# CAS-CLab/quantized-cnn

Measured on AMD Instinct MI355X. Metric: images/sec AlexNet quantized forward, higher is better.
Workload: dtype f32

## Files before the change

include/qcnn_hip.h:

```cpp
#ifndef QCNN_HIP_H_
#define QCNN_HIP_H_

#include <stddef.h>
#include <stdint.h>

#ifdef __cplusplus
extern "C" {
#endif

#define QCNN_ABI_VERSION 5

#define QCNN_SMALL_BATCH_MAX 3

typedef struct QcnnCtx QcnnCtx;

enum { QCNN_CONV = 0, QCNN_POOL = 1, QCNN_FCNT = 2, QCNN_RELU = 3, QCNN_LORN = 4, QCNN_DRPT = 5, QCNN_SMAX = 6 };

typedef struct {
  int type;
  int padSiz, knlSiz, knlCnt, grpCnt, stride, nodCnt, lrnSiz;
  float lrnAlp, lrnBet, lrnIni, drpRat;
} QcnnLayerDesc;

enum {
  QCNN_OPT_LUT_MODE = 0,
  QCNN_OPT_KEEP_ALL = 1,
  QCNN_OPT_PROFILE = 2,
  QCNN_OPT_SMALL_BATCH = 4,
  QCNN_OPT_SPLIT = 5,
  QCNN_OPT_SLIDE = 7,
  QCNN_OPT_DECODE = 8,
  QCNN_OPT_SYM = 9,
  QCNN_OPT_SYM8 = 10,
  QCNN_OPT_PACKED_FC = 11,
  QCNN_OPT_DIRECT_DEC = 12,
  QCNN_OPT_HALF8 = 13,
  QCNN_OPT_DEC_BF16SPLIT = 14,
  QCNN_OPT_HOST_CHUNK = 6,
  QCNN_OPT_STREAMS = 3
};

int qcnn_ctx_create(int device_id, void* stream, QcnnCtx** out);
int qcnn_ctx_destroy(QcnnCtx* ctx);
const char* qcnn_last_error(const QcnnCtx* ctx);
int qcnn_abi_version(void);
int qcnn_device_count(int* count);
int qcnn_set_option(QcnnCtx* ctx, int option, int value);
int qcnn_sync(QcnnCtx* ctx);
int qcnn_ctx_device(const QcnnCtx* ctx);
void* qcnn_ctx_stream(const QcnnCtx* ctx);

int qcnn_model_begin(QcnnCtx* ctx, int layer_cnt, const QcnnLayerDesc* layers, int in_c, int in_h, int in_w);
int qcnn_model_set_layer_shape(QcnnCtx* ctx, int layer, int M, int K, int Cs);
int qcnn_model_set_layer_dense(QcnnCtx* ctx, int layer);
int qcnn_model_set_layer_weights(QcnnCtx* ctx, int layer, const float* bias, const float* weights_file);
int qcnn_quantize_layer(QcnnCtx* ctx, int Ct, int Cin, int kh, int kw, int M, int K, int Cs, const float* weights_host,
                        const float* ctrd_init_host, int max_iter, float* ctrd_out_host, uint8_t* asmt_out_host, double* sse2,
                        int* iters2);
int qcnn_calib_gram(QcnnCtx* ctx, int H, int W, int Cin_total, int grp, int kh, int kw, int stride, int pad,
                    const float* in_nhwc_host, int n, double* gram_inout_host, int accumulate);
int qcnn_quantize_layer_ec(QcnnCtx* ctx, int Ct, int Cin, int grp, int kh, int kw, int M, int K, int Cs, const float* weights_host,
                           const double* gram_host, const float* ctrd_init_host, const uint8_t* asmt_init_host, int sweeps,
                           double ridge, float* ctrd_out_host, uint8_t* asmt_out_host, double* obj_trace, int* changed_trace);
int qcnn_calib_begin(QcnnCtx* ctx, const int* layers, int n_layers);
int qcnn_calib_arm(QcnnCtx* ctx, int on);
int qcnn_calib_read(QcnnCtx* ctx, int layer, double* gram_host, long long* rows);
int qcnn_calib_end(QcnnCtx* ctx);
int qcnn_model_arena_bytes(QcnnCtx* ctx, size_t* bytes);
int qcnn_model_commit(QcnnCtx* ctx, int max_batch, void* dev_arena);
int qcnn_model_arena_ptr(QcnnCtx* ctx, void** dev_ptr, size_t* bytes);
int qcnn_model_arena_checksum(QcnnCtx* ctx, unsigned long long* sum2);
int qcnn_model_set_layer_params(QcnnCtx* ctx, int layer, const float* bias, const float* ctrd_file,
                                const uint8_t* asmt_file);
int qcnn_model_set_layer_params_cbn(QcnnCtx* ctx, int layer, const float* bias, const float* ctrd_file,
                                    const uint8_t* cbn_blocks, size_t cbn_bytes, int bits);
int qcnn_model_mark_loaded(QcnnCtx* ctx);
int qcnn_fm_dims(QcnnCtx* ctx, int l, int* hwc3);

int qcnn_forward(QcnnCtx* ctx, const float* in_nchw_dev, int n, float* prob_dev, uint16_t* top5_dev);
int qcnn_forward_u8(QcnnCtx* ctx, const uint8_t* in_u8_dev, int src_h, int src_w, const float* mean_dev, int n,
                    float* prob_dev, uint16_t* top5_dev);
#define QCNN_MAX_VIEWS 32
typedef struct { int oy, ox, flip; } QcnnView;
int qcnn_views_ten_crop(int src_h, int src_w, int in_h, int in_w, QcnnView* views10);
int qcnn_forward_u8_views(QcnnCtx* ctx, const uint8_t* in_u8_dev, int src_h, int src_w, const float* mean_dev, int n,
                          const QcnnView* views_host, int n_views, float* prob_dev, uint16_t* top5_dev,
                          float* prob_views_dev );
typedef struct { uint64_t offset; int32_t h, w; } QcnnSrcImage;
int qcnn_forward_u8_resized_views(QcnnCtx* ctx, const uint8_t* src_dev, size_t src_bytes,
                                  const QcnnSrcImage* imgs_host, int n, int full_h, int full_w,
                                  const float* mean_dev ,
                                  const QcnnView* views_host, int n_views,
                                  float* prob_dev, uint16_t* top5_dev, float* prob_views_dev);
int qcnn_relaxed_full_size(int h, int w, int full_h, int full_w, int* hf, int* wf, float* scale);
typedef struct { int ay, ax, dy, dx, flip; } QcnnAnchorView;
int qcnn_views_ten_crop_anchored(QcnnAnchorView* views10);
int qcnn_forward_u8_relaxed_views(QcnnCtx* ctx, const uint8_t* src_dev, size_t src_bytes, const QcnnSrcImage* imgs_host, int n,
                                  int full_h, int full_w, const float* mean_crop_dev ,
                                  const QcnnAnchorView* views_host, int n_views,
                                  float* prob_dev, uint16_t* top5_dev, float* prob_views_dev);
typedef struct {
  uint64_t offset;
  int64_t  row_stride;
  int32_t  h, w;
  int32_t  pix_stride;
  int32_t  ch_offset[4];
} QcnnSrcPixels;
int qcnn_src_planar(const QcnnSrcImage* img, int C, QcnnSrcPixels* out);
int qcnn_src_bmp(const uint8_t* file_host, size_t file_bytes, uint64_t file_offset, QcnnSrcPixels* out);
int qcnn_forward_u8_resized_views_strided(QcnnCtx* ctx, const uint8_t* src_dev, size_t src_bytes,
                                          const QcnnSrcPixels* imgs_host, int n, int full_h, int full_w,
                                          const float* mean_dev ,
                                          const QcnnView* views_host, int n_views,
                                          float* prob_dev, uint16_t* top5_dev, float* prob_views_dev);
int qcnn_forward_u8_relaxed_views_strided(QcnnCtx* ctx, const uint8_t* src_dev, size_t src_bytes,
                                          const QcnnSrcPixels* imgs_host, int n, int full_h, int full_w,
                                          const float* mean_crop_dev ,
                                          const QcnnAnchorView* views_host, int n_views,
                                          float* prob_dev, uint16_t* top5_dev, float* prob_views_dev);
enum { QCNN_YUV_JFIF = 0, QCNN_YUV_BT601 = 1, QCNN_YUV_BT709 = 2 };
typedef struct {
  uint64_t y_offset, cb_offset, cr_offset;
  int64_t  y_row_stride, c_row_stride;
  int32_t  h, w;
  int32_t  y_pix_stride, c_pix_stride;
  int32_t  sub_y, sub_x;
  int32_t  matrix;
} QcnnSrcYuv;
enum { QCNN_YUV_NV12 = 0, QCNN_YUV_NV21 = 1, QCNN_YUV_I420 = 2, QCNN_YUV_YV12 = 3, QCNN_YUV_I444 = 4, QCNN_YUV_YUY2 = 5, QCNN_YUV_UYVY = 6 };
int qcnn_src_yuv_frame(int format, uint64_t frame_offset, int h, int w, int64_t pitch, int matrix, QcnnSrcYuv* out);
// ... 85 lines not shown
```

quantized-cnn_amd/capi.py:

```python
from __future__ import annotations

import ctypes as C
import os
import re

PKG = os.path.dirname(os.path.abspath(__file__))
LIB_PATH = os.environ.get("QCNN_HIP_LIB") or os.path.join(PKG, "libqcnn_hip.so")
HEADER_PATH = os.path.join(os.path.dirname(PKG), "include", "qcnn_hip.h")

OPT_LUT_MODE, OPT_KEEP_ALL, OPT_PROFILE, OPT_STREAMS, OPT_SMALL_BATCH, OPT_SPLIT, OPT_HOST_CHUNK, OPT_SLIDE, OPT_DECODE, OPT_SYM, OPT_SYM8, OPT_PACKED_FC, OPT_DIRECT_DEC, OPT_HALF8, OPT_DEC_BF16SPLIT = 0, 1, 2, 3, 4, 5, 6, 7, 8, 9, 10, 11, 12, 13, 14
LUT_EXACT, LUT_MFMA, LUT_MFMA_F16, LUT_MFMA_F16ACC = 0, 1, 2, 3
SMALL_BATCH_MAX = 3


class QcnnLayerDesc(C.Structure):
    _fields_ = [("type", C.c_int), ("padSiz", C.c_int), ("knlSiz", C.c_int), ("knlCnt", C.c_int),
                ("grpCnt", C.c_int), ("stride", C.c_int), ("nodCnt", C.c_int), ("lrnSiz", C.c_int),
                ("lrnAlp", C.c_float), ("lrnBet", C.c_float), ("lrnIni", C.c_float), ("drpRat", C.c_float)]


MAX_VIEWS = 32


class QcnnView(C.Structure):
# ... 27 lines not shown
    _fields_ = [("src_host", C.c_void_p), ("src_bytes", C.c_size_t), ("imgs", C.POINTER(QcnnSrcPixels)), ("n", C.c_int),
                ("labels", C.c_void_p), ("prob_host", C.c_void_p), ("top5_host", C.c_void_p), ("prob_views_host", C.c_void_p)]


class QcnnU8YuvBatch(C.Structure):
    _fields_ = [("src_host", C.c_void_p), ("src_bytes", C.c_size_t), ("imgs", C.POINTER(QcnnSrcYuv)), ("n", C.c_int),
                ("labels", C.c_void_p), ("prob_host", C.c_void_p), ("top5_host", C.c_void_p), ("prob_views_host", C.c_void_p)]


def layer_desc(ly: dict) -> QcnnLayerDesc:
    return QcnnLayerDesc(ly["type"], ly.get("pad", 0), ly.get("knl", 0), ly.get("cnt", 0), ly.get("grp", 0),
                         ly.get("stride", 0), ly.get("nod", 0), ly.get("siz", 0), ly.get("alp", 0.0),
                         ly.get("bet", 0.0), ly.get("ini", 0.0), ly.get("rat", 0.0))


def declared_symbols():
    txt = open(HEADER_PATH).read()
    txt = re.sub(r"/\*.*?\*/", "", txt, flags=re.S)
    return sorted(set(re.findall(r"\b(qcnn_[a-z0-9_]+)\s*\(", txt)))


_lib = None


def load():
    global _lib
    if _lib is not None:
        return _lib
    if not os.path.exists(LIB_PATH):
        raise RuntimeError("%s is missing: run `python -c 'import __graft_entry__ as g; g.build()'` "
                           "(hipcc --offload-arch=gfx950); there is no fallback path" % LIB_PATH)
    lib = C.CDLL(LIB_PATH)
    vp, i, f32p, u8p, u16p = C.c_void_p, C.c_int, C.c_void_p, C.c_void_p, C.c_void_p
    lib.qcnn_abi_version.restype = i
    lib.qcnn_device_count.argtypes = [C.POINTER(i)]
    lib.qcnn_last_error.restype = C.c_char_p
    lib.qcnn_last_error.argtypes = [vp]
    lib.qcnn_ctx_create.argtypes = [i, vp, C.POINTER(vp)]
    lib.qcnn_ctx_destroy.argtypes = [vp]
    lib.qcnn_set_option.argtypes = [vp, i, i]
    lib.qcnn_sync.argtypes = [vp]
    lib.qcnn_model_begin.argtypes = [vp, i, C.POINTER(QcnnLayerDesc), i, i, i]
    lib.qcnn_model_set_layer_shape.argtypes = [vp, i, i, i, i]
    lib.qcnn_model_set_layer_dense.argtypes = [vp, i]
    lib.qcnn_model_set_layer_weights.argtypes = [vp, i, f32p, f32p]
    lib.qcnn_group_model_set_layer_dense.argtypes = [vp, i]
    lib.qcnn_group_model_set_layer_weights.argtypes = [vp, i, f32p, f32p]
    lib.qcnn_model_arena_bytes.argtypes = [vp, C.POINTER(C.c_size_t)]
    lib.qcnn_model_commit.argtypes = [vp, i, vp]
    lib.qcnn_model_set_layer_params.argtypes = [vp, i, f32p, f32p, u8p]
    lib.qcnn_model_set_layer_params_cbn.argtypes = [vp, i, f32p, f32p, u8p, C.c_size_t, i]
    lib.qcnn_model_mark_loaded.argtypes = [vp]
    lib.qcnn_fm_dims.argtypes = [vp, i, C.POINTER(i)]
    lib.qcnn_forward.argtypes = [vp, f32p, i, f32p, u16p]
    lib.qcnn_forward_u8.argtypes = [vp, u8p, i, i, f32p, i, f32p, u16p]
    lib.qcnn_views_ten_crop.argtypes = [i, i, i, i, C.POINTER(QcnnView)]
    lib.qcnn_forward_u8_views.argtypes = [vp, u8p, i, i, f32p, i, C.POINTER(QcnnView), i, f32p, u16p, f32p]
    lib.qcnn_forward_u8_resized_views.argtypes = [vp, u8p, C.c_size_t, C.POINTER(QcnnSrcImage), i, i, i, f32p, C.POINTER(QcnnView), i,
                                                  f32p, u16p, f32p]
    lib.qcnn_views_ten_crop_anchored.argtypes = [C.POINTER(QcnnAnchorView)]
    lib.qcnn_relaxed_full_size.argtypes = [i, i, i, i, C.POINTER(i), C.POINTER(i), C.POINTER(C.c_float)]
    lib.qcnn_forward_u8_relaxed_views.argtypes = [vp, u8p, C.c_size_t, C.POINTER(QcnnSrcImage), i, i, i, f32p, C.POINTER(QcnnAnchorView), i,
                                                  f32p, u16p, f32p]
    lib.qcnn_src_planar.argtypes = [C.POINTER(QcnnSrcImage), i, C.POINTER(QcnnSrcPixels)]
    lib.qcnn_src_bmp.argtypes = [C.c_char_p, C.c_size_t, C.c_uint64, C.POINTER(QcnnSrcPixels)]
    lib.qcnn_forward_u8_resized_views_strided.argtypes = [vp, u8p, C.c_size_t, C.POINTER(QcnnSrcPixels), i, i, i, f32p,
                                                          C.POINTER(QcnnView), i, f32p, u16p, f32p]
    lib.qcnn_forward_u8_relaxed_views_strided.argtypes = [vp, u8p, C.c_size_t, C.POINTER(QcnnSrcPixels), i, i, i, f32p,
                                                          C.POINTER(QcnnAnchorView), i, f32p, u16p, f32p]
    lib.qcnn_src_yuv_frame.argtypes = [i, C.c_uint64, i, i, C.c_int64, i, C.POINTER(QcnnSrcYuv)]
    lib.qcnn_forward_u8_resized_views_yuv.argtypes = [vp, u8p, C.c_size_t, C.POINTER(QcnnSrcYuv), i, i, i, f32p, C.POINTER(QcnnView), i,
                                                      f32p, u16p, f32p]
    lib.qcnn_forward_u8_relaxed_views_yuv.argtypes = [vp, u8p, C.c_size_t, C.POINTER(QcnnSrcYuv), i, i, i, f32p,
                                                      C.POINTER(QcnnAnchorView), i, f32p, u16p, f32p]
    lib.qcnn_forward_host.argtypes = [vp, f32p, i, f32p, u16p]
    lib.qcnn_forward_host_batches.argtypes = [vp, C.POINTER(vp), C.POINTER(i), i, C.POINTER(vp), C.POINTER(vp)]
    lib.qcnn_forward_u8_resized_host_batches.argtypes = [vp, C.POINTER(QcnnU8Batch), i, i, i, f32p, C.POINTER(QcnnView), i,
                                                         C.POINTER(C.c_ulonglong)]
    lib.qcnn_forward_u8_relaxed_host_batches.argtypes = [vp, C.POINTER(QcnnU8Batch), i, i, i, f32p, C.POINTER(QcnnAnchorView), i,
                                                         C.POINTER(C.c_ulonglong)]
    lib.qcnn_forward_u8_resized_host_batches_yuv.argtypes = [vp, C.POINTER(QcnnU8YuvBatch), i, i, i, f32p, C.POINTER(QcnnView), i,
                                                             C.POINTER(C.c_ulonglong)]
    lib.qcnn_forward_u8_relaxed_host_batches_yuv.argtypes = [vp, C.POINTER(QcnnU8YuvBatch), i, i, i, f32p, C.POINTER(QcnnAnchorView), i,
                                                             C.POINTER(C.c_ulonglong)]
    lib.qcnn_count_top5_hits.argtypes = [vp, u16p, u16p, i, vp]
    lib.qcnn_host_register.argtypes = [vp, C.c_size_t]
    lib.qcnn_host_unregister.argtypes = [vp]
    lib.qcnn_host_alloc.argtypes = [C.c_size_t, C.POINTER(vp)]
    lib.qcnn_host_free.argtypes = [vp]
    lib.qcnn_get_layer_output.argtypes = [vp, i, i, f32p]
    lib.qcnn_get_layer_output_range.argtypes = [vp, i, i, i, f32p]
    lib.qcnn_run_layer.argtypes = [vp, i, f32p, i, f32p]
    lib.qcnn_get_layer_split.argtypes = [vp, i, C.POINTER(i), C.POINTER(i)]
    lib.qcnn_get_layer_dec_form.argtypes = [vp, i, C.POINTER(i), C.POINTER(C.c_longlong)]
    lib.qcnn_get_layer_segments.argtypes = [vp, i, C.POINTER(i), C.POINTER(i)]
    lib.qcnn_get_layer_ms.argtypes = [vp, C.POINTER(C.c_float), C.POINTER(i)]
    lib.qcnn_reset_layer_ms.argtypes = [vp]
    lib.qcnn_get_layer_total_ms.argtypes = [vp, C.POINTER(C.c_double), C.POINTER(C.c_longlong), C.POINTER(i)]
    lib.qcnn_ctx_device.argtypes = [vp]
    lib.qcnn_ctx_stream.argtypes = [vp]
    lib.qcnn_ctx_stream.restype = vp
    lib.qcnn_model_arena_ptr.argtypes = [vp, C.POINTER(vp), C.POINTER(C.c_size_t)]
    lib.qcnn_model_arena_checksum.argtypes = [vp, C.POINTER(C.c_ulonglong)]
    lib.qcnn_quantize_layer.argtypes = [vp, i, i, i, i, i, i, i, f32p, f32p, i, f32p, u8p, C.POINTER(C.c_double), C.POINTER(i)]
    lib.qcnn_calib_gram.argtypes = [vp, i, i, i, i, i, i, i, i, f32p, i, vp, i]
    lib.qcnn_calib_begin.argtypes = [vp, C.POINTER(i), i]
# ... 28 lines not shown
```

quantized-cnn_amd/csrc/qcnn_engine_run.hip:

```cpp
#include <stdlib.h>
#include <string.h>

#include <algorithm>

#include "qcnn_engine.h"

using namespace qcnn_engine;

namespace {

bool decoded_layer(const QcnnCtx* c, int l) {
  const LayerShape& s = c->shapes[l];
  return c->decode && s.decKp > 0 && !s.dense && c->lutMode == 1 && c->layers[l].type == QCNN_CONV;
}

int launched(QcnnCtx* c, int l, hipError_t e) {
  if (e != hipSuccess) return fail(c, "layer %d (type %d) launch failed: %s", l, c->layers[l].type, hipGetErrorString(e));
  return 0;
}

float* conv_partial(QcnnCtx* c, const Launch& L) {
  float* all = ensure_conv_partial(c);
  return all ? all + kConvPartialFloats / (size_t)L.nsub * L.sub : nullptr;
}
// ... 353 lines not shown
      if (prof) {
        HIP_TRY(c, hipEventRecord(e1, st));
        c->profPending.push_back(QcnnCtx::ProfRec{(((size_t)c->profCount * kMaxStreams + k) * c->L + l) * 2, l});
      }
    }
  }
  for (int k = 1; k < ns; ++k) {
    HIP_TRY(c, hipEventRecord(c->evJoin[k - 1], c->aux[k - 1]));
    HIP_TRY(c, hipStreamWaitEvent(c->stream, c->evJoin[k - 1], 0));
  }
  if (c->calib.armed && calib_enqueue(c, fm, n, pa, pb)) return 1;
  if (prof) c->profCount++;
  if (pa == 0 || (int)c->lastFm.size() != c->L + 1) {
    c->lastFm = fm;
  } else {
    for (int l = 0; l <= c->L; ++l)
      if (fm[l] == nullptr) c->lastFm[l] = nullptr;
  }
  c->lastN = n;
  return 0;
}

int map_outputs(QcnnCtx* c, const float* map, int n, float* prob_dev, uint16_t* top5_dev) {
  const int classes = (int)fm_elems(c, c->L);
  hipError_t e;
  if (prob_dev) {
    e = qk_unpack_rows(map, prob_dev, n, classes, c->stream);
    if (e != hipSuccess) return fail(c, "output unpack launch failed: %s", hipGetErrorString(e));
  }
  if (top5_dev) {
    e = qk_top5(map, top5_dev, n, classes, c->stream);
    if (e != hipSuccess) return fail(c, "top-5 launch failed: %s", hipGetErrorString(e));
  }
  return 0;
}
int forward_outputs(QcnnCtx* c, int n, float* prob_dev, uint16_t* top5_dev) {
  return map_outputs(c, c->lastFm[c->L], n, prob_dev, top5_dev);
}
int forward_tail(QcnnCtx* c, int n, float* prob_dev, uint16_t* top5_dev, const float* inNchw) {
  if (run_layers(c, n, inNchw)) return 1;
  return forward_outputs(c, n, prob_dev, top5_dev);
}

}

extern "C" {

int qcnn_fm_dims(QcnnCtx* c, int l, int* hwc3) {
  if (l < 0 || l > c->L) return fail(c, "feature map %d out of range", l);
  hwc3[0] = c->dims[l].h; hwc3[1] = c->dims[l].w; hwc3[2] = c->dims[l].c;
  return 0;
}

int qcnn_forward(QcnnCtx* c, const float* in_nchw_dev, int n, float* prob_dev, uint16_t* top5_dev) {
  if (open_batch(c, n)) return 1;
  if (direct_input(c, n)) return forward_tail(c, n, prob_dev, top5_dev, in_nchw_dev);
  hipError_t e = qk_pack_nchw(in_nchw_dev, c->fmBuf[0], n, c->inC, c->inH, c->inW, c->stream);
  if (e != hipSuccess) return fail(c, "input pack launch failed: %s", hipGetErrorString(e));
  return forward_tail(c, n, prob_dev, top5_dev);
}

int qcnn_forward_u8(QcnnCtx* c, const uint8_t* in_u8_dev, int src_h, int src_w, const float* mean_dev, int n,
                    float* prob_dev, uint16_t* top5_dev) {
  if (open_batch(c, n)) return 1;
  if (src_h < c->inH || src_w < c->inW)
    return fail(c, "source images %dx%d are smaller than the network input %dx%d", src_h, src_w, c->inH, c->inW);
  hipError_t e = qk_pack_u8(in_u8_dev, mean_dev, c->fmBuf[0], n, c->inC, c->inH, c->inW, src_h, src_w, c->stream);
  if (e != hipSuccess) return fail(c, "input pack launch failed: %s", hipGetErrorString(e));
  return forward_tail(c, n, prob_dev, top5_dev);
}

int qcnn_get_layer_output(QcnnCtx* c, int l, int n, float* host_out) {
  HIP_TRY(c, hipSetDevice(c->device));
  if (l < 0 || l > c->L) return fail(c, "feature map %d out of range", l);
  if (n <= 0 || n > c->lastN) return fail(c, "n = %d exceeds the last forward's batch %d", n, c->lastN);
  if (layer_output_ok(c, l)) return 1;
  if (ensure_stage(c, (size_t)n * fm_elems(c, l))) return 1;
  const int E = (int)fm_elems(c, l);
  hipError_t e = qk_unpack_rows(c->lastFm[l], c->stageOut, n, E, c->stream);
  if (e != hipSuccess) return fail(c, "unpack launch failed: %s", hipGetErrorString(e));
  HIP_TRY(c, hipMemcpyAsync(host_out, c->stageOut, (size_t)n * E * sizeof(float), hipMemcpyDeviceToHost, c->stream));
  HIP_TRY(c, hipStreamSynchronize(c->stream));
  return 0;
}

int qcnn_get_layer_output_range(QcnnCtx* c, int l, int first, int n, float* host_out) {
  HIP_TRY(c, hipSetDevice(c->device));
  if (l < 0 || l > c->L) return fail(c, "feature map %d out of range", l);
  if (first < 0 || n <= 0 || first + n > c->lastN)
    return fail(c, "images [%d, %d) are not inside the last forward's batch of %d", first, first + n, c->lastN);
  if (layer_output_ok(c, l)) return 1;
  if (ensure_stage(c, (size_t)(n + QCNN_PANEL) * fm_elems(c, l))) return 1;
  const size_t E = fm_elems(c, l);
  const int p0 = first / QCNN_PANEL;
  const int cnt = first + n - p0 * QCNN_PANEL;
  hipError_t e = qk_unpack_rows(c->lastFm[l] + (size_t)p0 * E * QCNN_PANEL, c->stageOut, cnt, (int)E, c->stream);
  if (e != hipSuccess) return fail(c, "unpack launch failed: %s", hipGetErrorString(e));
  HIP_TRY(c, hipMemcpyAsync(host_out, c->stageOut + (size_t)(first - p0 * QCNN_PANEL) * E, (size_t)n * E * sizeof(float),
                            hipMemcpyDeviceToHost, c->stream));
  HIP_TRY(c, hipStreamSynchronize(c->stream));
  return 0;
}

int qcnn_run_layer(QcnnCtx* c, int layer, const float* in_host, int n, float* out_host) {
  HIP_TRY(c, hipSetDevice(c->device));
  if (!c->committed) return fail(c, "model not committed");
// ... 98 lines not shown
```

quantized-cnn_amd/csrc/qcnn_glue.hip:

```cpp
#include "qcnn_kernels.h"

#include <float.h>
#include <limits.h>

#include <algorithm>

typedef float f32x2 __attribute__((ext_vector_type(2)));
typedef float f32x4 __attribute__((ext_vector_type(4)));

namespace {

constexpr int PANEL = QCNN_PANEL;

__global__ void k_permute_rows(const float* __restrict__ src, float* __restrict__ dst, const int* __restrict__ map,
                               int D, int panels, int livePairs) {
  const int lane = threadIdx.x & 63;
  if (lane >= livePairs) return;
  const size_t rows = (size_t)panels * D;
  for (size_t r = blockIdx.x * (size_t)(blockDim.x >> 6) + (threadIdx.x >> 6); r < rows;
       r += (size_t)gridDim.x * (blockDim.x >> 6)) {
    const size_t panel = r / D;
    const int e = (int)(r % D);
    *reinterpret_cast<f32x2*>(dst + r * PANEL + 2 * lane) =
        *reinterpret_cast<const f32x2*>(src + (panel * D + map[e]) * PANEL + 2 * lane);
  }
}

__global__ void k_sum_partials(const float4* __restrict__ partial, float4* __restrict__ dst, int msplit, size_t n4,
                               int relu) {
  for (size_t i = blockIdx.x * (size_t)blockDim.x + threadIdx.x; i < n4; i += (size_t)gridDim.x * blockDim.x) {
    float4 v = partial[i];
    for (int z = 1; z < msplit; ++z) {
      const float4 w = partial[(size_t)z * n4 + i];
      v.x += w.x; v.y += w.y; v.z += w.z; v.w += w.w;
    }
    if (relu) {
      v.x = (0.0f < v.x) ? v.x : 0.0f;
      v.y = (0.0f < v.y) ? v.y : 0.0f;
      v.z = (0.0f < v.z) ? v.z : 0.0f;
      v.w = (0.0f < v.w) ? v.w : 0.0f;
    }
    dst[i] = v;
  }
}

__global__ void k_relu(const float4* __restrict__ src, float4* __restrict__ dst, size_t n4) {
  for (size_t i = blockIdx.x * (size_t)blockDim.x + threadIdx.x; i < n4; i += (size_t)gridDim.x * blockDim.x) {
    float4 v = src[i];
    v.x = (0.0f < v.x) ? v.x : 0.0f;
    v.y = (0.0f < v.y) ? v.y : 0.0f;
    v.z = (0.0f < v.z) ? v.z : 0.0f;
    v.w = (0.0f < v.w) ? v.w : 0.0f;
    dst[i] = v;
  }
}

template <bool B34>
__device__ __forceinline__ float lrn_scale(float s, float nbet) {
  if (B34) {
    const float r = __builtin_amdgcn_rsqf(s);
    return __fmul_rn(r, __builtin_amdgcn_sqrtf(r));
  }
  return expf(__fmul_rn(nbet, logf(s)));
}

// ... 90 lines not shown
    const int wL = max(0, wo * stride - pad), wU = min(W, wo * stride + knl - pad) - 1;
    const float* base = src + (size_t)panel * H * W * C * PANEL + 2 * lane;
    f32x2 v = {0.0f, 0.0f};
    bool first = true;
    for (int h = hL; h <= hU; ++h)
      for (int w = wL; w <= wU; ++w) {
        const f32x2 s = *reinterpret_cast<const f32x2*>(base + ((size_t)(h * W + w) * C + c) * PANEL);
        if (first) {
          v = s;
        } else {
          v.x = (s.x < v.x) ? v.x : s.x;
          v.y = (s.y < v.y) ? v.y : s.y;
        }
        first = false;
      }
    *reinterpret_cast<f32x2*>(dst + r * PANEL + 2 * lane) = v;
  }
}

__global__ __launch_bounds__(256) void k_pool4(const float4* __restrict__ src, float4* __restrict__ dst, int panels,
                                               int H, int W, int C, int Ho, int Wo, int knl, int stride, int pad,
                                               int liveQuads, int qlShift) {
  const size_t rows = (size_t)panels * Ho * Wo * C;
  const size_t r = (blockIdx.x * (size_t)blockDim.x + threadIdx.x) >> qlShift;
  const int q = threadIdx.x & ((1 << qlShift) - 1);
  if (r >= rows || q >= liveQuads) return;
  const int c = (int)(r % C);
  size_t t = r / C;
  const int wo = (int)(t % Wo);
  t /= Wo;
  const int ho = (int)(t % Ho);
  const int panel = (int)(t / Ho);
  const int hL = max(0, ho * stride - pad), hU = min(H, ho * stride + knl - pad) - 1;
  const int wL = max(0, wo * stride - pad), wU = min(W, wo * stride + knl - pad) - 1;
  const float4* base = src + (size_t)panel * H * W * C * 32 + q;
  float4 v = make_float4(0.0f, 0.0f, 0.0f, 0.0f);
  bool first = true;
  for (int h = hL; h <= hU; ++h)
    for (int w = wL; w <= wU; ++w) {
      const float4 sv = base[((size_t)(h * W + w) * C + c) * 32];
      if (first) {
        v = sv;
      } else {
        v.x = (sv.x < v.x) ? v.x : sv.x;
        v.y = (sv.y < v.y) ? v.y : sv.y;
        v.z = (sv.z < v.z) ? v.z : sv.z;
        v.w = (sv.w < v.w) ? v.w : sv.w;
      }
      first = false;
    }
  dst[r * 32 + q] = v;
}

#ifndef QCNN_LP_PREFETCH
#define QCNN_LP_PREFETCH 0
#endif
#ifndef QCNN_LP_PT
#define QCNN_LP_PT 4
#define QCNN_LP_Q 8
#define QCNN_LP_THREADS 704
#endif
constexpr int LP_PT = QCNN_LP_PT;
constexpr int LP_IT = (LP_PT - 1) * 2 + 3;
constexpr int LP_PIX = LP_IT * LP_IT;
constexpr int LP_Q = QCNN_LP_Q;
constexpr int LP_THREADS = QCNN_LP_THREADS;
template <int N, bool B34>
__global__ __launch_bounds__(LP_THREADS, QCNN_LP_PREFETCH ? 2 : 1) void k_lrn_pool(const float4* __restrict__ src, float4* __restrict__ dst, int H,
                                                         int W, int C, int Ho, int Wo, int tilesX, float coeff, float nbet,
                                                         float ini, int liveQuads) {
  constexpr int RAD = (N - 1) / 2;
  __shared__ float4 slab[N * LP_PIX * LP_Q];
  const int q = threadIdx.x & (LP_Q - 1), rest = threadIdx.x / LP_Q;
  const int slices = 32 / LP_Q;
  const int slice = blockIdx.x % slices, tile = blockIdx.x / slices;
  const int panel = blockIdx.y;
  const int qg = slice * LP_Q + q;
  const bool qlive = qg < liveQuads;
  const int ty = tile / tilesX, tx = tile % tilesX;
  const int ph = ty * LP_PT * 2 + rest / LP_IT, pw = tx * LP_PT * 2 + rest % LP_IT;
  const bool lrnOn = rest < LP_PIX && ph < H && pw < W && qlive;
  const float4* __restrict__ x = src + ((size_t)panel * H * W + (size_t)(lrnOn ? ph * W + pw : 0)) * C * 32 + qg;
  const int pu = rest % N, po = rest / N;
  const int ho = ty * LP_PT + po / LP_PT, wo = tx * LP_PT + po % LP_PT;
  const bool poolOn = po < LP_PT * LP_PT && ho < Ho && wo < Wo && qlive;
  const int hU = min(H, ho * 2 + 3) - 1 - ty * LP_PT * 2, wU = min(W, wo * 2 + 3) - 1 - tx * LP_PT * 2;
  const int hL = (po / LP_PT) * 2, wL = (po % LP_PT) * 2;
  float4* __restrict__ y = dst + ((size_t)panel * Ho * Wo + (size_t)(poolOn ? ho * Wo + wo : 0)) * C * 32 + qg;

  const f32x4 zero = {0.0f, 0.0f, 0.0f, 0.0f};
  f32x4 raw[N], sq[N];
#pragma unroll
  for (int j = 0; j < N; ++j) { raw[j] = zero; sq[j] = zero; }
#pragma unroll
  for (int d = -RAD; d < RAD; ++d) {
    const bool on = lrnOn && d >= 0 && d < C;
    const f32x4 v = ld4(x + (size_t)(on ? d : 0) * 32, on);
    raw[(d + N) % N] = v;
    sq[(d + N) % N] = lrn_sq(v, coeff);
  }
  f32x4* __restrict__ slab4 = reinterpret_cast<f32x4*>(slab);
#if QCNN_LP_PREFETCH
  f32x4 nxt[N];
#pragma unroll
  for (int u = 0; u < N; ++u) nxt[u] = ld4(x + (size_t)(u + RAD < C ? u + RAD : 0) * 32, lrnOn && u + RAD < C);
#endif
  for (int c0 = 0; c0 < C; c0 += N) {
    if (lrnOn) {
#pragma unroll
      for (int u = 0; u < N; ++u) {
        const int c = c0 + u;
        const int tin = c + RAD;
#if QCNN_LP_PREFETCH
        const f32x4 v = nxt[u];
        {
          const int tn = c0 + N + u + RAD;
          nxt[u] = ld4(x + (size_t)(tn < C ? tn : 0) * 32, tn < C);
        }
#else
        const f32x4 v = ld4(x + (size_t)(tin < C ? tin : 0) * 32, tin < C);
#endif
        raw[(u + RAD) % N] = v;
        sq[(u + RAD) % N] = lrn_sq(v, coeff);
        if (c < C) {
          f32x4 sacc = {ini, ini, ini, ini};
#pragma unroll
          for (int j = 0; j < N; ++j) sacc = sacc + sq[(u - RAD + j + N) % N];
          slab4[(u * LP_PIX + rest) * LP_Q + q] = lrn_out<B34>(raw[u % N], sacc, nbet);
        }
      }
    }
    __syncthreads();
    if (poolOn && c0 + pu < C) {
      float4 v = make_float4(0.0f, 0.0f, 0.0f, 0.0f);
      bool first = true;
      for (int h = hL; h <= hU; ++h)
        for (int w = wL; w <= wU; ++w) {
          const float4 sv = slab[(pu * LP_PIX + h * LP_IT + w) * LP_Q + q];
          if (first) {
            v = sv;
          } else {
            v.x = (sv.x < v.x) ? v.x : sv.x;
            v.y = (sv.y < v.y) ? v.y : sv.y;
            v.z = (sv.z < v.z) ? v.z : sv.z;
            v.w = (sv.w < v.w) ? v.w : sv.w;
          }
          first = false;
        }
      y[(size_t)(c0 + pu) * 32] = v;
    }
    __syncthreads();
  }
}

constexpr int SM_LD = 33;
__global__ __launch_bounds__(1024) void k_softmax_lds(const float* __restrict__ src, float* __restrict__ dst, int C) {
  extern __shared__ __attribute__((aligned(16))) char lds[];
  float* tile = reinterpret_cast<float*>(lds);
  float* sums = tile + (size_t)C * SM_LD;
  const int img = threadIdx.x & 31, cl = threadIdx.x >> 5;
  const size_t off = (size_t)blockIdx.y * C * PANEL + blockIdx.x * 32 + img;
  const float* x = src + off;
  float* y = dst + off;
  int c = cl;
  for (; c + 96 < C; c += 128) {
    const float v0 = x[(size_t)c * PANEL], v1 = x[(size_t)(c + 32) * PANEL], v2 = x[(size_t)(c + 64) * PANEL],
                v3 = x[(size_t)(c + 96) * PANEL];
    tile[c * SM_LD + img] = expf(v0);
    tile[(c + 32) * SM_LD + img] = expf(v1);
    tile[(c + 64) * SM_LD + img] = expf(v2);
    tile[(c + 96) * SM_LD + img] = expf(v3);
  }
  for (; c < C; c += 32) tile[c * SM_LD + img] = expf(x[(size_t)c * PANEL]);
  __syncthreads();
  if (cl == 0) {
    float sum = 0.0f;
    int k = 0;
    for (; k + 16 <= C; k += 16) {
      float v[16];
#pragma unroll
      for (int j = 0; j < 16; ++j) v[j] = tile[(k + j) * SM_LD + img];
#pragma unroll
      for (int j = 0; j < 16; ++j) sum = __fadd_rn(sum, v[j]);
    }
    for (; k < C; ++k) sum = __fadd_rn(sum, tile[k * SM_LD + img]);
    sums[img] = sum;
  }
  __syncthreads();
  const float sum = sums[img];
  for (c = cl; c < C; c += 32) y[(size_t)c * PANEL] = __fdiv_rn(tile[c * SM_LD + img], sum);
}

__global__ __launch_bounds__(1024) void k_top5_lds(const float* __restrict__ prob, uint16_t* __restrict__ out, int n,
                                                   int C) {
  extern __shared__ __attribute__((aligned(16))) char lds[];
  float* tile = reinterpret_cast<float*>(lds);
  {
    const int img = threadIdx.x & 31, cl = threadIdx.x >> 5;
    const float* x = prob + (size_t)blockIdx.y * C * PANEL + blockIdx.x * 32 + img;
    int c = cl;
    for (; c + 96 < C; c += 128) {
      const float v0 = x[(size_t)c * PANEL], v1 = x[(size_t)(c + 32) * PANEL], v2 = x[(size_t)(c + 64) * PANEL],
                  v3 = x[(size_t)(c + 96) * PANEL];
      tile[c * SM_LD + img] = v0;
      tile[(c + 32) * SM_LD + img] = v1;
      tile[(c + 64) * SM_LD + img] = v2;
      tile[(c + 96) * SM_LD + img] = v3;
// ... 235 lines not shown
  return hipGetLastError();
}

hipError_t qk_permute_rows(const float* src, float* dst, const int* map, int D, int panels, int live, hipStream_t st) {
  const size_t rows = (size_t)panels * D;
  const int blocks = (int)((rows + 3) / 4 < 8192 ? (rows + 3) / 4 : 8192);
  hipLaunchKernelGGL(k_permute_rows, dim3(blocks ? blocks : 1), dim3(256), 0, st, src, dst, map, D, panels, (live + 1) / 2);
  return hipGetLastError();
}

hipError_t qk_relu(const float* src, float* dst, size_t n, hipStream_t st) {
  const size_t n4 = n / 4;
  const int blocks = (int)((n4 + 255) / 256 < 4096 ? (n4 + 255) / 256 : 4096);
  hipLaunchKernelGGL(k_relu, dim3(blocks ? blocks : 1), dim3(256), 0, st, reinterpret_cast<const float4*>(src),
                     reinterpret_cast<float4*>(dst), n4);
  return hipGetLastError();
}

namespace {
int live_shift(int live) {
  const int quads = (live + 3) / 4;
  int s = 0;
  while ((1 << s) < quads) ++s;
  return s > 5 ? 5 : s;
}
}

hipError_t qk_lrn(const float* src, float* dst, int panels, int HW, int C, int lrnSiz, float alp, float bet, float ini,
                  int live, hipStream_t st) {
  const size_t rows = (size_t)panels * HW * C;
  const float coeff = alp / lrnSiz;
  if (lrnSiz == 5 || lrnSiz == 3) {
    const size_t pixels = (size_t)panels * HW;
    const int qlShift = live_shift(live);
    const size_t blocks = ((pixels << qlShift) + 255) / 256;
    int segs = (int)std::min<size_t>((2048 + blocks - 1) / blocks, (size_t)std::max(1, C / ((qlShift < 5 ? 2 : 4) * lrnSiz)));
    int segLen = ((C + segs - 1) / segs + lrnSiz - 1) / lrnSiz * lrnSiz;
    segs = (C + segLen - 1) / segLen;
    const dim3 grid((unsigned)blocks, (unsigned)segs);
    auto kern = k_lrn_stream<5, false>;
    if (lrnSiz == 5) kern = (bet == 0.75f) ? k_lrn_stream<5, true> : k_lrn_stream<5, false>;
    else kern = (bet == 0.75f) ? k_lrn_stream<3, true> : k_lrn_stream<3, false>;
    hipLaunchKernelGGL(kern, grid, dim3(256), 0, st, reinterpret_cast<const float4*>(src),
                       reinterpret_cast<float4*>(dst), pixels, C, segLen, coeff, -bet, ini, (live + 3) / 4, qlShift);
    return hipGetLastError();
  }
  const int blocks = (int)((rows + 3) / 4 < 8192 ? (rows + 3) / 4 : 8192);
  hipLaunchKernelGGL(k_lrn, dim3(blocks ? blocks : 1), dim3(256), 0, st, src, dst, rows, C, lrnSiz, coeff, -bet, ini);
  return hipGetLastError();
}

int qk_lrn_pool_blocks(int Ho, int Wo) { return ((Ho + LP_PT - 1) / LP_PT) * ((Wo + LP_PT - 1) / LP_PT) * (32 / LP_Q); }

hipError_t qk_lrn_pool(const float* src, float* dst, int panels, int H, int W, int C, int Ho, int Wo, int lrnSiz, float alp,
                       float bet, float ini, int live, hipStream_t st) {
  if (lrnSiz != 5 && lrnSiz != 3) return hipErrorInvalidValue;
  const float coeff = alp / lrnSiz;
  const int tilesX = (Wo + LP_PT - 1) / LP_PT;
  const dim3 grid((unsigned)qk_lrn_pool_blocks(Ho, Wo), (unsigned)panels);
  auto kern = k_lrn_pool<5, false>;
  if (lrnSiz == 5) kern = (bet == 0.75f) ? k_lrn_pool<5, true> : k_lrn_pool<5, false>;
  else kern = (bet == 0.75f) ? k_lrn_pool<3, true> : k_lrn_pool<3, false>;
  hipLaunchKernelGGL(kern, grid, dim3(LP_THREADS), 0, st, reinterpret_cast<const float4*>(src),
                     reinterpret_cast<float4*>(dst), H, W, C, Ho, Wo, tilesX, coeff, -bet, ini, (live + 3) / 4);
  return hipGetLastError();
}

hipError_t qk_pool(const float* src, float* dst, int panels, int H, int W, int C, int Ho, int Wo, int knl, int stride,
                   int pad, int live, hipStream_t st) {
  const size_t rows = (size_t)panels * Ho * Wo * C;
  if ((rows + 7) / 8 < (size_t)1 << 31) {
    const int qlShift = live_shift(live);
    hipLaunchKernelGGL(k_pool4, dim3((unsigned)(((rows << qlShift) + 255) / 256)), dim3(256), 0, st,
                       reinterpret_cast<const float4*>(src), reinterpret_cast<float4*>(dst), panels, H, W, C, Ho, Wo, knl,
                       stride, pad, (live + 3) / 4, qlShift);
    return hipGetLastError();
  }
  const int blocks = (int)((rows + 3) / 4 < 8192 ? (rows + 3) / 4 : 8192);
  hipLaunchKernelGGL(k_pool, dim3(blocks ? blocks : 1), dim3(256), 0, st, src, dst, panels, H, W, C, Ho, Wo, knl,
                     stride, pad);
  return hipGetLastError();
}

hipError_t qk_softmax(const float* src, float* dst, int panels, int C, int live, hipStream_t st) {
  const size_t shm = ((size_t)C * SM_LD + 32) * sizeof(float);
  if (shm <= 160 * 1024) {
    hipError_t e = hipFuncSetAttribute(reinterpret_cast<const void*>(k_softmax_lds),
                                       hipFuncAttributeMaxDynamicSharedMemorySize, (int)shm);
    if (e != hipSuccess) return e;
    hipLaunchKernelGGL(k_softmax_lds, dim3((live + 31) / 32, panels), dim3(1024), shm, st, src, dst, C);
    return hipGetLastError();
  }
  hipLaunchKernelGGL(k_softmax, dim3((panels * PANEL + 63) / 64), dim3(64), 0, st, src, dst, panels, C);
  return hipGetLastError();
}

hipError_t qk_top5(const float* prob, uint16_t* out, int n, int C, hipStream_t st) {
  const size_t shm = (size_t)C * SM_LD * sizeof(float);
  if (shm <= 160 * 1024) {
    hipError_t e = hipFuncSetAttribute(reinterpret_cast<const void*>(k_top5_lds),
                                       hipFuncAttributeMaxDynamicSharedMemorySize, (int)shm);
    if (e != hipSuccess) return e;
    hipLaunchKernelGGL(k_top5_lds, dim3(n <= PANEL ? (n + 31) / 32 : PANEL / 32, panels_of(n)), dim3(1024), shm, st, prob, out, n, C);
    return hipGetLastError();
  }
  hipLaunchKernelGGL(k_top5, dim3((n + 63) / 64), dim3(64), 0, st, prob, out, n, C);
  return hipGetLastError();
}

hipError_t qk_top5_hits(const uint16_t* top5, const uint16_t* labels, int n, unsigned long long* hits5, hipStream_t st) {
  if (n <= 0 || !top5 || !labels || !hits5) return hipErrorInvalidValue;
  hipLaunchKernelGGL(k_top5_hits, dim3((n + HITS_BLOCK - 1) / HITS_BLOCK), dim3(HITS_BLOCK), 0, st, top5, labels, n, hits5);
// ... 66 lines not shown
```

quantized-cnn_amd/csrc/qcnn_kernels.h:

```cpp
#ifndef QCNN_KERNELS_H_
#define QCNN_KERNELS_H_

#include <hip/hip_runtime.h>
#include <stdint.h>

#define QCNN_PANEL 128
#define QCNN_MAX_CS 8
#define QCNN_MAX_K 128
#define QCNN_MAX_K_FILE 256
#define QCNN_ROWS_PAD 256
#define QCNN_STAGE_ROWS 128
#define QCNN_TILE_BYTES 8192
#define QCNN_STAGE_BYTES (8 * QCNN_TILE_BYTES)
#define QCNN_GATHER_WAVES 12
constexpr int NW8 = 8;
constexpr int FC8_CPW = 96;
constexpr int FC8_SUBB = NW8 * 2 * (FC8_CPW / 2) * 2;

__host__ __device__ static inline int qcnn_stage_group(int K) { return K <= 64 ? QCNN_STAGE_ROWS / K : 1; }
__host__ __device__ static inline int qcnn_row_slot(int r) { return (r & 0x70) | ((r & 3) << 2) | ((r >> 2) & 3); }
__host__ __device__ static inline uint16_t qcnn_row_offset(int r) { return (uint16_t)(qcnn_row_slot(r) * 64); }

struct QkSlots {
  int cpw;
// ... 178 lines not shown
  float* dst;
  const float* bias;
  const float* ctrd;
  const uint8_t* rows;
  const uint8_t* cbn;
  int cbnBits;
  int D, Ct, M, Cs, K;
  int pd;
  int relu;
  int panels;
  int lutF16;
};

bool qk_fc_sym8_shape(int D, int Ct, int M, int Cs, int K);
int qk_fc_sym8_chunks(int Ct);
size_t qk_fc_sym8_program_bytes(int Ct, int M);
hipError_t qk_build_program_fc8(const uint8_t* rows, uint16_t* prog, const QkSlots& src, int Ct, int M, hipStream_t st, int f16 = 0);
hipError_t qk_fc_sym8(const FcParams& p, const uint16_t* prog, const float* ctrdF, hipStream_t st, int mode = 0);
__host__ __device__ static inline size_t qk_ctrdf_index(int m, int d, int k) {
  const int stage = m >> 2, rt = 2 * (m & 3) + (k >> 4), h = rt >> 2, i = rt & 3, li = k & 15;
  return ((((size_t)stage * 2 + h) * 64) + d * 16 + li) * 4 + i;
}

struct DenseParams {
  const float* src;
  float* dst;
  const float* bias;
  const float* wt;
  int H, W, Cin, Ho, Wo, Ct;
  int knl, stride, pad, grp;
  int relu;
  int panels;
};
hipError_t qk_dense(const DenseParams& p, hipStream_t st);

hipError_t qk_conv_aprx(const ConvParams& p, int lutMode, hipStream_t st);
hipError_t qk_fc_aprx(const FcParams& p, int lutMode, hipStream_t st);
hipError_t qk_conv_small(const ConvParams& p, int n, hipStream_t st);
hipError_t qk_fc_small(const FcParams& p, int n, hipStream_t st);

hipError_t qk_decode_cbn(const uint8_t* blocks, int bits, size_t n, int Ct, int taps, int M, int K, QkSlots sl,
                         uint8_t* rows, int* bad, hipStream_t st);

hipError_t qk_build_program(const uint8_t* rows, uint16_t* prog, QkSlots src, QkSlots dst, QkProgram pg, int knl, int stride,
                            int M, hipStream_t st, int slide = 0);

hipError_t qk_permute_rows(const float* src, float* dst, const int* map, int D, int panels, int live, hipStream_t st);
hipError_t qk_sum_partials(const float* partial, float* dst, int msplit, size_t n, int relu, hipStream_t st);

hipError_t qk_relu(const float* src, float* dst, size_t n, hipStream_t st);
hipError_t qk_lrn(const float* src, float* dst, int panels, int HW, int C, int lrnSiz, float alp, float bet,
                  float ini, int live, hipStream_t st);
int qk_lrn_pool_blocks(int Ho, int Wo);
hipError_t qk_lrn_pool(const float* src, float* dst, int panels, int H, int W, int C, int Ho, int Wo, int lrnSiz, float alp,
                       float bet, float ini, int live, hipStream_t st);
hipError_t qk_pool(const float* src, float* dst, int panels, int H, int W, int C, int Ho, int Wo, int knl,
                   int stride, int pad, int live, hipStream_t st);
struct DecParams {
  int srcNchw;
  int nImages, panel0;
  const float* src;
  float* dst;
  const float* bias;
  const float* wdec;
  int H, W, Cin, Ho, Wo, Ct;
  int knl, stride, pad;
  int Kr, Kp, S;
  int relu, panels, live;
  float accScale, outScale;
  uint32_t* guard;
  uint32_t epoch;
};
bool qk_conv_dec_shape(int Cin, int grp, int M, int Ct, int knl, int* Kp, int* S);
hipError_t qk_decode_weights(const uint8_t* rows, const float* ctrd, float* out, const QkSlots& sl, int knl, int Cin, int K,
                             int Ct, int Kp, int S, hipStream_t st);
hipError_t qk_conv_dec(const DecParams& p, hipStream_t st);
bool qk_conv_dec_nchw_shape(int Cin, int grp, int M, int Ct, int knl, int pad, int* Kp);
hipError_t qk_decode_weights_nchw(const uint8_t* rows, const float* ctrd, float* out, const QkSlots& sl, int knl, int Cin, int K,
                                  int Ct, int Kp, int S, hipStream_t st);
hipError_t qk_conv_dec_nchw(const DecParams& p, hipStream_t st);
bool qk_conv_dec_nchw_split_shape(int Cin, int grp, int M, int Ct, int knl, int pad, int* Kb);
hipError_t qk_decode_weights_split(const uint8_t* rows, const float* ctrd, uint16_t* out, const QkSlots& sl, int knl, int Cin, int K,
                                   int Ct, int Kb, hipStream_t st);
hipError_t qk_conv_dec_nchw_split(const DecParams& p, hipStream_t st);
#define QK_F16_SX 64.0f
#define QK_F16_XMAX 1023.0f
#define QK_F16_PLANES 256
__host__ __device__ inline float qk_f16_weight_scale(uint32_t maxW, uint32_t maxBias) {
  const int e = (int)(maxW >> 23) - 127;
  if (maxW >= 0x7f800000u || maxW < 0x00800000u || e < -107 || e > 19 || maxBias >= 0x7f800000u) return 0.0f;
  const uint32_t swBits = (uint32_t)(13 - e + 127) << 23, limBits = (uint32_t)(100 + 127) << 23;
  float Sw = 0.0f, b = 0.0f, lim = 0.0f;
  __builtin_memcpy(&Sw, &swBits, 4); __builtin_memcpy(&b, &maxBias, 4); __builtin_memcpy(&lim, &limBits, 4);
  return b * (QK_F16_SX * Sw) <= lim ? Sw : 0.0f;
}
size_t qk_conv_dec_nchw_f16_bytes(int Kb, int Ct);
size_t qk_conv_dec_nchw_f16_guard_bytes(int Ho, int Wo, int Ct, int panels);
hipError_t qk_decode_weights_f16(const uint8_t* rows, const float* ctrd, const float* bias, void* out, const QkSlots& sl, int knl,
                                 int Cin, int K, int Ct, int Kb, hipStream_t st);
hipError_t qk_conv_dec_nchw_f16(const DecParams& p, const float* wBf16, hipStream_t st);
struct FcDecParams {
  const float* src;
  float* dst;
  float* partial;
  const float* bias;
  const float* wdec;
// ... 83 lines not shown
```

Measured before the change: 111,100.

## Add ring-buffered async-LDS LRN+pool kernel with reordered pixel slots

Adds a new fused LRN+maxpool kernel that streams channel slices into a D-deep LDS ring via direct global-to-LDS loads, waiting on vmcnt per slot so loads of later channels overlap LRN compute and pooling of earlier ones. Pixels are permuted into parity-interleaved LDS positions to reduce bank conflicts in the 3x3 pool reads. It becomes the default path for LRN sizes 3/5 when the panel fits 32-bit offsets, replacing the register-prefetch variant. It costs more dynamic LDS (lower occupancy) and adds two barriers per chunk.

```diff
diff --git a/include/qcnn_hip.h b/include/qcnn_hip.h
--- a/include/qcnn_hip.h
+++ b/include/qcnn_hip.h
@@ -76,6 +76,7 @@
                                     const uint8_t* cbn_blocks, size_t cbn_bytes, int bits);
 int qcnn_model_mark_loaded(QcnnCtx* ctx);
 int qcnn_fm_dims(QcnnCtx* ctx, int l, int* hwc3);
+int qcnn_lrn_pool_ring(int lrn_siz, int c, int h, int w);
 
 int qcnn_forward(QcnnCtx* ctx, const float* in_nchw_dev, int n, float* prob_dev, uint16_t* top5_dev);
 int qcnn_forward_u8(QcnnCtx* ctx, const uint8_t* in_u8_dev, int src_h, int src_w, const float* mean_dev, int n,
diff --git a/quantized-cnn_amd/capi.py b/quantized-cnn_amd/capi.py
--- a/quantized-cnn_amd/capi.py
+++ b/quantized-cnn_amd/capi.py
@@ -103,6 +103,8 @@
     lib.qcnn_model_set_layer_params_cbn.argtypes = [vp, i, f32p, f32p, u8p, C.c_size_t, i]
     lib.qcnn_model_mark_loaded.argtypes = [vp]
     lib.qcnn_fm_dims.argtypes = [vp, i, C.POINTER(i)]
+    if hasattr(lib, "qcnn_lrn_pool_ring"):
+        lib.qcnn_lrn_pool_ring.argtypes = [i, i, i, i]
     lib.qcnn_forward.argtypes = [vp, f32p, i, f32p, u16p]
     lib.qcnn_forward_u8.argtypes = [vp, u8p, i, i, f32p, i, f32p, u16p]
     lib.qcnn_views_ten_crop.argtypes = [i, i, i, i, C.POINTER(QcnnView)]
diff --git a/quantized-cnn_amd/csrc/qcnn_engine_run.hip b/quantized-cnn_amd/csrc/qcnn_engine_run.hip
--- a/quantized-cnn_amd/csrc/qcnn_engine_run.hip
+++ b/quantized-cnn_amd/csrc/qcnn_engine_run.hip
@@ -429,6 +429,8 @@
   return 0;
 }
 
+int qcnn_lrn_pool_ring(int lrn_siz, int c, int h, int w) { return qk_lrn_pool_ring(h, w, c, lrn_siz); }
+
 int qcnn_forward(QcnnCtx* c, const float* in_nchw_dev, int n, float* prob_dev, uint16_t* top5_dev) {
   if (open_batch(c, n)) return 1;
   if (direct_input(c, n)) return forward_tail(c, n, prob_dev, top5_dev, in_nchw_dev);
diff --git a/quantized-cnn_amd/csrc/qcnn_glue.hip b/quantized-cnn_amd/csrc/qcnn_glue.hip
--- a/quantized-cnn_amd/csrc/qcnn_glue.hip
+++ b/quantized-cnn_amd/csrc/qcnn_glue.hip
@@ -1,16 +1,12 @@
-#include "qcnn_kernels.h"
+#include "qcnn_dev.h"
 
 #include <float.h>
 #include <limits.h>
 
 #include <algorithm>
-
-typedef float f32x2 __attribute__((ext_vector_type(2)));
-typedef float f32x4 __attribute__((ext_vector_type(4)));
+#include <type_traits>
 
 namespace {
-
-constexpr int PANEL = QCNN_PANEL;
 
 __global__ void k_permute_rows(const float* __restrict__ src, float* __restrict__ dst, const int* __restrict__ map,
                                int D, int panels, int livePairs) {
@@ -207,9 +203,6 @@
   dst[r * 32 + q] = v;
 }
 
-#ifndef QCNN_LP_PREFETCH
-#define QCNN_LP_PREFETCH 0
-#endif
 #ifndef QCNN_LP_PT
 #define QCNN_LP_PT 4
 #define QCNN_LP_Q 8
@@ -221,9 +214,9 @@
 constexpr int LP_Q = QCNN_LP_Q;
 constexpr int LP_THREADS = QCNN_LP_THREADS;
 template <int N, bool B34>
-__global__ __launch_bounds__(LP_THREADS, QCNN_LP_PREFETCH ? 2 : 1) void k_lrn_pool(const float4* __restrict__ src, float4* __restrict__ dst, int H,
-                                                         int W, int C, int Ho, int Wo, int tilesX, float coeff, float nbet,
-                                                         float ini, int liveQuads) {
+__global__ __launch_bounds__(LP_THREADS, 1) void k_lrn_pool(const float4* __restrict__ src, float4* __restrict__ dst, int H, int W, int C,
+                                                            int Ho, int Wo, int tilesX, float coeff, float nbet, float ini,
+                                                            int liveQuads) {
   constexpr int RAD = (N - 1) / 2;
   __shared__ float4 slab[N * LP_PIX * LP_Q];
   const int q = threadIdx.x & (LP_Q - 1), rest = threadIdx.x / LP_Q;
@@ -255,26 +248,13 @@
     sq[(d + N) % N] = lrn_sq(v, coeff);
   }
   f32x4* __restrict__ slab4 = reinterpret_cast<f32x4*>(slab);
-#if QCNN_LP_PREFETCH
-  f32x4 nxt[N];
-#pragma unroll
-  for (int u = 0; u < N; ++u) nxt[u] = ld4(x + (size_t)(u + RAD < C ? u + RAD : 0) * 32, lrnOn && u + RAD < C);
-#endif
   for (int c0 = 0; c0 < C; c0 += N) {
     if (lrnOn) {
 #pragma unroll
       for (int u = 0; u < N; ++u) {
         const int c = c0 + u;
         const int tin = c + RAD;
-#if QCNN_LP_PREFETCH
-        const f32x4 v = nxt[u];
-        {
-          const int tn = c0 + N + u + RAD;
-          nxt[u] = ld4(x + (size_t)(tn < C ? tn : 0) * 32, tn < C);
-        }
-#else
         const f32x4 v = ld4(x + (size_t)(tin < C ? tin : 0) * 32, tin < C);
-#endif
         raw[(u + RAD) % N] = v;
         sq[(u + RAD) % N] = lrn_sq(v, coeff);
         if (c < C) {
@@ -308,6 +288,159 @@
   }
 }
 
+constexpr int LP_SLOT = LP_PIX * LP_Q;
+struct LpOrder {
+  unsigned char posOf[LP_PIX];
+  unsigned char pixAt[LP_PIX];
+};
+constexpr LpOrder lp_order() {
+  static_assert(LP_PIX <= 255, "positions are bytes");
+  LpOrder o{};
+  int next[2] = {0, 1};
+  for (int p = 0; p < LP_PIX; ++p) {
+    int par = ((p / LP_IT >> 1) + (p % LP_IT >> 1)) & 1;
+    if (next[par] >= LP_PIX) par ^= 1;
+    o.posOf[p] = (unsigned char)next[par];
+    o.pixAt[next[par]] = (unsigned char)p;
+    next[par] += 2;
+  }
+  return o;
+}
+__constant__ const LpOrder lpOrder = lp_order();
+
+template <int K>
+__device__ __forceinline__ void lp_wait_vm() { asm volatile("s_waitcnt vmcnt(%0)" :: "n"(K) : "memory"); }
+__device__ __forceinline__ void lp_wait_vm(int n) {
+  if (n >= 8) lp_wait_vm<8>();
+  else if (n >= 4) lp_wait_vm<4>();
+  else if (n >= 2) lp_wait_vm<2>();
+  else if (n == 1) lp_wait_vm<1>();
+  else lp_wait_vm<0>();
+}
+
+template <int B, int E, class F>
+__device__ __forceinline__ void lp_for(F&& f) {
+  if constexpr (B < E) {
+    f(std::integral_constant<int, B>{});
+    lp_for<B + 1, E>(f);
+  }
+}
+
+template <int N, bool B34, int D>
+__global__ __launch_bounds__(LP_THREADS, 1) void k_lrn_pool_ring(const float4* __restrict__ src, float4* __restrict__ dst, int H, int W,
+                                                                 int C, int Ho, int Wo, int tilesX, float coeff, float nbet,
+                                                                 float ini, int liveQuads) {
+  constexpr int RAD = (N - 1) / 2;
+  static_assert(D >= N && D <= 16, "a chunk's N slots are live together; vmcnt counts D - 1 DMAs");
+  static_assert(LP_THREADS % 64 == 0 && LP_Q == 8, "a wave-instruction of the DMA = 8 positions x 8 quads");
+  extern __shared__ __attribute__((aligned(16))) float4 lpRing[];
+  f32x4* __restrict__ ring4 = reinterpret_cast<f32x4*>(lpRing);
+  const int tid = threadIdx.x;
+  const int q = tid & (LP_Q - 1), rest = tid / LP_Q;
+  const int slices = 32 / LP_Q;
+  const int slice = blockIdx.x % slices, tile = blockIdx.x / slices;
+  const int panel = blockIdx.y;
+  const int qg = slice * LP_Q + q;
+  const bool qlive = qg < liveQuads;
+  const int ty = tile / tilesX, tx = tile % tilesX;
+  const int pix = lpOrder.pixAt[rest < LP_PIX ? rest : 0];
+  const int ph = ty * LP_PT * 2 + pix / LP_IT, pw = tx * LP_PT * 2 + pix % LP_IT;
+  const bool lrnOn = rest < LP_PIX && ph < H && pw < W && qlive;
+  const char* __restrict__ panelBase = reinterpret_cast<const char*>(src + (size_t)panel * H * W * C * 32);
+  const uint32_t xoff = lrnOn ? ((uint32_t)(ph * W + pw) * (uint32_t)C * 32u + (uint32_t)qg) * 16u : 0u;
+  const uint32_t ldsWave = (uint32_t)uni((int)(uint32_t)(size_t)lpRing + (tid >> 6) * 1024);
+  const int pu = rest % N, po = rest / N;
+  const int ho = ty * LP_PT + po / LP_PT, wo = tx * LP_PT + po % LP_PT;
+  const bool poolOn = po < LP_PT * LP_PT && ho < Ho && wo < Wo && qlive;
+  const int hU = min(H, ho * 2 + 3) - 1 - ty * LP_PT * 2, wU = min(W, wo * 2 + 3) - 1 - tx * LP_PT * 2;
+  const int hL = (po / LP_PT) * 2, wL = (po % LP_PT) * 2;
+  int win[9];
+#pragma unroll
+  for (int i = 0; i < 3; ++i)
+#pragma unroll
+    for (int j = 0; j < 3; ++j) win[i * 3 + j] = lpOrder.posOf[poolOn ? (hL + i) * LP_IT + wL + j : 0] * LP_Q + q;
+  float4* __restrict__ y = dst + ((size_t)panel * Ho * Wo + (size_t)(poolOn ? ho * Wo + wo : 0)) * C * 32 + qg;
+
+  int issued = 0, issSlot = 0;
+  auto issue_to = [&](int hi) {
+    hi = min(hi, C);
+    for (; issued < hi; ++issued) {
+      if (lrnOn) glds16(panelBase + (size_t)issued * 512, xoff, ldsWave + (uint32_t)issSlot * (uint32_t)(LP_SLOT * 16));
+      issSlot = issSlot + 1 == D ? 0 : issSlot + 1;
+    }
+  };
+  issue_to(D);
+
+  const f32x4 zero = {0.0f, 0.0f, 0.0f, 0.0f};
+  f32x4 raw[N], sq[N];
+#pragma unroll
+  for (int j = 0; j < N; ++j) { raw[j] = zero; sq[j] = zero; }
+#pragma unroll
+  for (int d = 0; d < RAD; ++d) {
+    f32x4 v = zero;
+    if (lrnOn && d < C) {
+      lp_wait_vm(issued - d - 1);
+      v = ring4[d * LP_SLOT + tid];
+    }
+    raw[d] = v;
+    sq[d] = lrn_sq(v, coeff);
+  }
+  asm volatile("s_waitcnt lgkmcnt(0)" ::: "memory");
+  int s0 = RAD;
+  for (int c0 = 0; c0 < C; c0 += N) {
+    issue_to(c0 + RAD + D);
+    const bool whole = c0 + RAD + D <= C;
+    if (lrnOn) {
+      lp_for<0, N>([&](auto uc) {
+        constexpr int u = decltype(uc)::value;
+        const int c = c0 + u;
+        const int tin = c + RAD;
+        const int st = s0 + u >= D ? s0 + u - D : s0 + u;
+        f32x4 v = zero;
+        if (tin < C) {
+          if (whole) lp_wait_vm<D - 1 - u>();
+          else lp_wait_vm(issued - tin - 1);
+          v = ring4[st * LP_SLOT + tid];
+        }
+        raw[(u + RAD) % N] = v;
+        sq[(u + RAD) % N] = lrn_sq(v, coeff);
+        if (c < C) {
+          f32x4 sacc = {ini, ini, ini, ini};
+#pragma unroll
+          for (int j = 0; j < N; ++j) sacc = sacc + sq[(u - RAD + j + N) % N];
+          ring4[st * LP_SLOT + tid] = lrn_out<B34>(raw[u % N], sacc, nbet);
+        }
+      });
+    }
+    barrier_after_lds_writes();
+    if (poolOn && c0 + pu < C) {
+      const int sp = s0 + pu;
+      const float4* __restrict__ slot = lpRing + (sp >= D ? sp - D : sp) * LP_SLOT;
+      float4 v = make_float4(0.0f, 0.0f, 0.0f, 0.0f);
+      bool first = true;
+#pragma unroll
+      for (int i = 0; i < 3; ++i)
+#pragma unroll
+        for (int j = 0; j < 3; ++j)
+          if (hL + i <= hU && wL + j <= wU) {
+            const float4 sv = slot[win[i * 3 + j]];
+            if (first) {
+              v = sv;
+            } else {
+              v.x = (sv.x < v.x) ? v.x : sv.x;
+              v.y = (sv.y < v.y) ? v.y : sv.y;
+              v.z = (sv.z < v.z) ? v.z : sv.z;
+              v.w = (sv.w < v.w) ? v.w : sv.w;
+            }
+            first = false;
+          }
+      y[(size_t)(c0 + pu) * 32] = v;
+    }
+    barrier_after_lds_writes();
+    s0 = s0 + N >= D ? s0 + N - D : s0 + N;
+  }
+}
+
 constexpr int SM_LD = 33;
 __global__ __launch_bounds__(1024) void k_softmax_lds(const float* __restrict__ src, float* __restrict__ dst, int C) {
   extern __shared__ __attribute__((aligned(16))) char lds[];
@@ -649,12 +782,49 @@
 
 int qk_lrn_pool_blocks(int Ho, int Wo) { return ((Ho + LP_PT - 1) / LP_PT) * ((Wo + LP_PT - 1) / LP_PT) * (32 / LP_Q); }
 
+constexpr int LP_RING = 7;
+int qk_lrn_pool_ring(int H, int W, int C, int lrnSiz) {
+  if (lrnSiz != 5 && lrnSiz != 3) return 0;
+  if ((unsigned long long)H * W * C * 512ull > 0xffffffffull) return 0;
+#ifdef QCNN_EXPERIMENT
+  static const int forced = [] { const char* e = getenv("QCNN_LP_RING"); return e ? atoi(e) : -1; }();
+  if (forced == 0 || forced == 10 || forced == 14) return forced;
+#endif
+  return LP_RING;
+}
+
+template <int N, bool B34, int D>
+hipError_t lrn_pool_ring_launch(dim3 grid, hipStream_t st, const float* src, float* dst, int H, int W, int C, int Ho, int Wo,
+                                int tilesX, float coeff, float nbet, float ini, int liveQuads) {
+  constexpr int bytes = D * LP_SLOT * 16;
+  static_assert(bytes <= 160 * 1024, "the ring fits the LDS of a CU");
+  const hipError_t e = allow_big_lds(reinterpret_cast<const void*>(k_lrn_pool_ring<N, B34, D>), bytes);
+  if (e != hipSuccess) return e;
+  hipLaunchKernelGGL((k_lrn_pool_ring<N, B34, D>), grid, dim3(LP_THREADS), bytes, st, reinterpret_cast<const float4*>(src),
+                     reinterpret_cast<float4*>(dst), H, W, C, Ho, Wo, tilesX, coeff, nbet, ini, liveQuads);
+  return hipGetLastError();
+}
+template <int D, class... A>
+hipError_t lrn_pool_ring_variant(int lrnSiz, bool b34, A... a) {
+  if (lrnSiz == 5) return b34 ? lrn_pool_ring_launch<5, true, D>(a...) : lrn_pool_ring_launch<5, false, D>(a...);
+  return b34 ? lrn_pool_ring_launch<3, true, D>(a...) : lrn_pool_ring_launch<3, false, D>(a...);
+}
+
 hipError_t qk_lrn_pool(const float* src, float* dst, int panels, int H, int W, int C, int Ho, int Wo, int lrnSiz, float alp,
                        float bet, float ini, int live, hipStream_t st) {
   if (lrnSiz != 5 && lrnSiz != 3) return hipErrorInvalidValue;
   const float coeff = alp / lrnSiz;
   const int tilesX = (Wo + LP_PT - 1) / LP_PT;
   const dim3 grid((unsigned)qk_lrn_pool_blocks(Ho, Wo), (unsigned)panels);
+  const int ring = qk_lrn_pool_ring(H, W, C, lrnSiz);
+  if (ring == LP_RING)
+    return lrn_pool_ring_variant<LP_RING>(lrnSiz, bet == 0.75f, grid, st, src, dst, H, W, C, Ho, Wo, tilesX, coeff, -bet, ini, (live + 3) / 4);
+#ifdef QCNN_EXPERIMENT
+  if (ring == 10)
+    return lrn_pool_ring_variant<10>(lrnSiz, bet == 0.75f, grid, st, src, dst, H, W, C, Ho, Wo, tilesX, coeff, -bet, ini, (live + 3) / 4);
+  if (ring == 14)
+    return lrn_pool_ring_variant<14>(lrnSiz, bet == 0.75f, grid, st, src, dst, H, W, C, Ho, Wo, tilesX, coeff, -bet, ini, (live + 3) / 4);
+#endif
   auto kern = k_lrn_pool<5, false>;
   if (lrnSiz == 5) kern = (bet == 0.75f) ? k_lrn_pool<5, true> : k_lrn_pool<5, false>;
   else kern = (bet == 0.75f) ? k_lrn_pool<3, true> : k_lrn_pool<3, false>;
diff --git a/quantized-cnn_amd/csrc/qcnn_kernels.h b/quantized-cnn_amd/csrc/qcnn_kernels.h
--- a/quantized-cnn_amd/csrc/qcnn_kernels.h
+++ b/quantized-cnn_amd/csrc/qcnn_kernels.h
@@ -254,6 +254,7 @@
 hipError_t qk_lrn(const float* src, float* dst, int panels, int HW, int C, int lrnSiz, float alp, float bet,
                   float ini, int live, hipStream_t st);
 int qk_lrn_pool_blocks(int Ho, int Wo);
+int qk_lrn_pool_ring(int H, int W, int C, int lrnSiz);
 hipError_t qk_lrn_pool(const float* src, float* dst, int panels, int H, int W, int C, int Ho, int Wo, int lrnSiz, float alp,
                        float bet, float ini, int live, hipStream_t st);
 hipError_t qk_pool(const float* src, float* dst, int panels, int H, int W, int C, int Ho, int Wo, int knl,
```

Result: no change. 111,700 (median of 6 runs) (+0.6%).
